# iwanders/spread_spectrum_watermarking

Measured on AMD Instinct MI355X. Metric: Mpixels/sec embed+extract (4K batch), higher is better.
Workload: dtype f64

## Files before the change

spread_spectrum_watermarking_amd/csrc/base_energy.hip:

```cpp
#include <algorithm>
#include <cmath>

#include "dct_pair_common.hpp"

namespace ssw {

namespace {

typedef _Float16 h8 __attribute__((ext_vector_type(8)));
typedef float f4 __attribute__((ext_vector_type(4)));

constexpr int BE_THREADS = 512, BE_LINES = 128;
constexpr int BE_NJ = 11;
constexpr float BE_BSCALE = 1024.0f;
constexpr unsigned BE_FRAG = 64 * 16;

struct BeClass {
    const double *x1, *x2;
    const u32x4* y16;
    const float* bmax;
    unsigned NP, Kp, pair0, pm, c1, c2, gsh, e2off, njt;
};
struct BeArgs {
    BeClass c[8];
    unsigned L, lpf, units_valid, W, chunks;
    float factor;
    float* energy;
};

__global__ __launch_bounds__(256) void base_energy_split_kernel(const double* __restrict__ y1, const double* __restrict__ y2, unsigned yrows,
                                                                unsigned NP, unsigned Kp, unsigned pair0, unsigned njt, size_t total,
                                                                _Float16* __restrict__ out, float* __restrict__ bmax) {
    const size_t idx = blockIdx.x * (size_t)blockDim.x + threadIdx.x;
    if (idx >= total) return;
    const unsigned e = (unsigned)(idx & 7u), lane = (unsigned)((idx >> 3) & 63u);
    size_t rest = idx >> 9;
    const unsigned j = (unsigned)(rest % njt);
    rest /= njt;
    const unsigned hl = (unsigned)(rest & 1u), p = (unsigned)((rest >> 1) & 1u), s = (unsigned)(rest >> 2);
    const unsigned pair = pair0 + 16u * j + (lane & 15u), k = 32u * s + 8u * (lane >> 4) + e;
    double b = 0.0;
    if (pair < NP && k < Kp) b = (p ? y2 : y1)[blk_index<double>(pair, k, yrows)];
    const float bf = (float)(b * (double)BE_BSCALE);
    const _Float16 h = (_Float16)bf;
    const float lo = bf - (float)h;
    out[idx] = hl ? (_Float16)lo : h;
    if (hl == 0 && b != 0.0) atomicMax(reinterpret_cast<unsigned*>(bmax), __float_as_uint(fabsf((float)b) * (1.0f + 0x1p-20f)));
}

__global__ __launch_bounds__(BE_THREADS) void prep16_row_energy_kernel(const BeArgs a) {
    __shared__ __attribute__((aligned(16))) u32x4 bsh[4 * BE_NJ * 64];
    __shared__ float eb[2][16 * BE_NJ];
    const unsigned tid = threadIdx.x, lane = tid & 63u, wave = tid >> 6, li = lane & 15u, lq = lane >> 4;
    const unsigned cls = blockIdx.y / a.chunks, chunk = blockIdx.y - cls * a.chunks;
    const BeClass& c = a.c[cls];
    const unsigned j0 = chunk * BE_NJ;
    if (j0 >= c.njt) return;
    const unsigned nj = c.njt - j0 < (unsigned)BE_NJ ? c.njt - j0 : (unsigned)BE_NJ;
    const unsigned m0 = blockIdx.x * BE_LINES, L = a.L;
    const unsigned z = m0 / a.lpf, unit = (m0 - z * a.lpf) / 16u + wave;
    const bool wave_valid = unit < a.units_valid && m0 + 16u * wave < L;
    const unsigned line = m0 + 16u * wave + li < L ? m0 + 16u * wave + li : L - 1u;
    const unsigned nkb = c.Kp / 8u, nsteps = (nkb + 3u) / 4u;
    for (unsigned i = tid; i < 2u * 16u * BE_NJ; i += BE_THREADS) (&eb[0][0])[i] = 0.f;

    const unsigned nq = 4u * nj * 64u;
    u32x4 breg[6];
    auto bload = [&](unsigned s) {
#pragma unroll
        for (int i = 0; i < 6; ++i) {
            const unsigned q = tid + BE_THREADS * i < nq ? tid + BE_THREADS * i : nq - 1u;
            const unsigned ph = q / (nj * 64u), rem = q - ph * (nj * 64u);
            breg[i] = c.y16[((size_t)(s * 4u + ph) * c.njt + j0) * 64u + rem];
        }
    };
    auto bstore = [&]() {
#pragma unroll
        for (int i = 0; i < 6; ++i) {
            const unsigned q = tid + BE_THREADS * i;
            if (q < nq) bsh[q] = breg[i];
        }
    };
    double2 araw[2][4];
    auto aload = [&](unsigned s) {
        const unsigned kb = 4u * s + lq;
#pragma unroll
        for (int o = 0; o < 2; ++o) {
            const double2* src = reinterpret_cast<const double2*>((o ? c.x2 : c.x1) + ((size_t)kb * L + line) * 8u);
#pragma unroll
            for (int i = 0; i < 4; ++i) araw[o][i] = kb < nkb ? src[i] : make_double2(0.0, 0.0);
        }
    };

    f4 acc[2][BE_NJ];
#pragma unroll
    for (int o = 0; o < 2; ++o)
#pragma unroll
        for (int j = 0; j < BE_NJ; ++j) acc[o][j] = (f4){0.f, 0.f, 0.f, 0.f};
    float S[2] = {0.f, 0.f};

    bload(0);
    aload(0);
    bstore();
    __syncthreads();
    for (unsigned s = 0; s < nsteps; ++s) {
        h8 xh[2], xl[2];
#pragma unroll
        for (int o = 0; o < 2; ++o)
#pragma unroll
            for (int i = 0; i < 4; ++i) {
                const float f0 = (float)araw[o][i].x, f1 = (float)araw[o][i].y;
                S[o] += fabsf(f0);
                S[o] += fabsf(f1);
                const _Float16 h0 = (_Float16)f0, h1 = (_Float16)f1;
                xh[o][2 * i] = h0; xh[o][2 * i + 1] = h1;
                xl[o][2 * i] = (_Float16)(f0 - (float)h0); xl[o][2 * i + 1] = (_Float16)(f1 - (float)h1);
            }
        if (s + 1 < nsteps) { bload(s + 1); aload(s + 1); }
        const h8* bf = reinterpret_cast<const h8*>(bsh);
#pragma unroll
        for (int j = 0; j < BE_NJ; ++j) {
            if ((unsigned)j < nj) {
#pragma unroll
            for (int o = 0; o < 2; ++o) {
                const h8 bh = bf[((2 * o) * nj + j) * 64u + lane], bl = bf[((2 * o + 1) * nj + j) * 64u + lane];
                f4 t = __builtin_amdgcn_mfma_f32_16x16x32_f16(xh[o], bl, (f4){0.f, 0.f, 0.f, 0.f}, 0, 0, 0);
                t = __builtin_amdgcn_mfma_f32_16x16x32_f16(xl[o], bh, t, 0, 0, 0);
                acc[o][j] = __builtin_amdgcn_mfma_f32_16x16x32_f16(xh[o], bh, acc[o][j], 0, 0, 0);
                acc[o][j] += t;
            }
            }
        }
        __syncthreads();
        if (s + 1 < nsteps) bstore();
        __syncthreads();
    }

#pragma unroll
    for (int o = 0; o < 2; ++o) { S[o] += __shfl_xor(S[o], 16); S[o] += __shfl_xor(S[o], 32); }
    const float k1 = 1.0f + 0x1p-20f;
    const float B = *c.bmax, n_ops = (float)(c.Kp + c.Kp / 16u + 16u);
    const float cS = (B * (3.0f * 0x1p-21f + 1.02f * n_ops * 0x1p-23f) + 0x1p-23f) * k1;
    const float cA = 1.01f * (float)c.Kp * B * 0x1p-13f * k1 + 1e-30f;
    float err[2][4];
#pragma unroll
    for (int o = 0; o < 2; ++o)
#pragma unroll
        for (int r = 0; r < 4; ++r) err[o][r] = (__shfl(S[o], (int)(4u * lq + r)) * cS + cA) * k1;
    const float fac = fabsf(a.factor) * k1;
#pragma unroll
    for (int j = 0; j < BE_NJ; ++j) {
        if ((unsigned)j >= nj) continue;
        float v1 = 0.f, v2 = 0.f;
#pragma unroll
        for (int r = 0; r < 4; ++r) {
            const float a1 = acc[0][j][r] * (1.0f / BE_BSCALE), a2 = acc[1][j][r] * (1.0f / BE_BSCALE);
            float o1, o2, e1, e2;
            if (c.pm) { o1 = fabsf(a1 + a2); o2 = fabsf(a1 - a2); e1 = e2 = err[0][r] + err[1][r]; }
            else      { o1 = fabsf(a1); o2 = fabsf(a2); e1 = err[0][r]; e2 = err[1][r]; }
            const float b1 = (o1 + e1) * k1 * fac, b2 = (o2 + e2) * k1 * fac;
            v1 += b1 * b1 * k1;
            v2 += b2 * b2 * k1;
        }
        v1 += __shfl_xor(v1, 16); v1 += __shfl_xor(v1, 32);
        v2 += __shfl_xor(v2, 16); v2 += __shfl_xor(v2, 32);
        if (wave_valid && lq == 0) {
            atomicAdd(&eb[0][16 * j + li], v1);
            atomicAdd(&eb[1][16 * j + li], v2);
        }
    }
    __syncthreads();
    if (tid < 2u * 16u * nj) {
        const unsigned o = tid / (16u * nj), pl = tid - o * (16u * nj);
        const unsigned pair = c.pair0 + 16u * j0 + pl;
        if (pair < c.NP && pair >= c.e2off * o) {
            const unsigned e = pair - (o ? c.e2off : 0u);
            const unsigned col = (o ? c.c2 : c.c1) + (e >> c.gsh) * 128u + (e & ((1u << c.gsh) - 1u));
            if (col < a.W) unsafeAtomicAdd(a.energy + (size_t)z * a.W + col, eb[o][pl]);
        }
    }
}

unsigned be_tiles(unsigned NP, unsigned pair0) { return NP > pair0 ? (NP - pair0 + 15u) / 16u : 0u; }
unsigned be_steps(unsigned Kp) { return (Kp / 8u + 3u) / 4u; }
size_t be_frag_bytes(unsigned NP, unsigned Kp, unsigned pair0) { return (size_t)be_steps(Kp) * 4u * be_tiles(NP, pair0) * BE_FRAG; }

}

size_t base_energy_split_bytes(unsigned NP, unsigned Kp, unsigned pair0) { return be_frag_bytes(NP, Kp, pair0) + 16; }

int launch_base_energy_split(hipStream_t st, const double* y1, const double* y2, unsigned yrows, unsigned NP, unsigned Kp, unsigned pair0, void* out) {
    const unsigned njt = be_tiles(NP, pair0);
    if (!y1 || !y2 || !out || njt == 0 || Kp == 0 || Kp % 8 != 0 || pair0 % 16 != 0 || yrows < NP) return SSW_ERR_BAD_ARG;
    const size_t frag = be_frag_bytes(NP, Kp, pair0), total = frag / sizeof(_Float16);
    float* bmax = reinterpret_cast<float*>(static_cast<char*>(out) + frag);
    SSW_HIP_CHECK(hipMemsetAsync(bmax, 0, 16, st));
    base_energy_split_kernel<<<(unsigned)((total + 255) / 256), 256, 0, st>>>(y1, y2, yrows, NP, Kp, pair0, njt, total, static_cast<_Float16*>(out), bmax);
    SSW_HIP_CHECK(hipGetLastError());
    return SSW_OK;
}

int launch_base_energy_bound(hipStream_t st, int n_classes, const BaseEnergyClass* cls, size_t n_frames, size_t w, size_t h, size_t lines_per_frame,
                             float factor, float* energy) {
    if (n_frames == 0 || n_classes == 0) return SSW_OK;
    const size_t lines = n_frames * lines_per_frame;
    if (n_classes < 0 || n_classes > 8 || !cls || !energy || lines_per_frame % BE_LINES != 0 || h % 16 != 0 || h > lines_per_frame ||
        lines > 0xFFFFFFFFull || w > 0xFFFFFFull || w % 128 != 0) return SSW_ERR_BAD_ARG;
    BeArgs a;
    unsigned chunks = 0;
    for (int i = 0; i < n_classes; ++i) {
        const BaseEnergyClass& s = cls[i];
        const unsigned njt = be_tiles(s.NP, s.pair0);
        if (!s.x1 || !s.x2 || !s.y16 || njt == 0 || s.Kp == 0 || s.Kp % 8 != 0 || s.pair0 % 16 != 0 || s.gsh > 16 || s.e2off > 1) return SSW_ERR_BAD_ARG;
        if ((unsigned long long)s.Kp * lines * sizeof(double) > 0xFFFFFFFFFFull) return SSW_ERR_BAD_DIMS;
        a.c[i] = BeClass{s.x1, s.x2, static_cast<const u32x4*>(s.y16),
                         reinterpret_cast<const float*>(static_cast<const char*>(s.y16) + be_frag_bytes(s.NP, s.Kp, s.pair0)),
                         s.NP, s.Kp, s.pair0, s.pm, s.c1, s.c2, s.gsh, s.e2off, njt};
        chunks = std::max(chunks, (njt + BE_NJ - 1) / BE_NJ);
    }
    a.L = (unsigned)lines; a.lpf = (unsigned)lines_per_frame; a.units_valid = (unsigned)(h / 16); a.W = (unsigned)w; a.chunks = chunks;
    a.factor = factor; a.energy = energy;
    const dim3 grid((unsigned)(lines / BE_LINES), (unsigned)n_classes * chunks);
    if (grid.y > 65535u) return SSW_ERR_BAD_DIMS;
    prep16_row_energy_kernel<<<grid, BE_THREADS, 0, st>>>(a);
    SSW_HIP_CHECK(hipGetLastError());
    return SSW_OK;
}

}
```

Baseline: 17680.

## Pipeline base-energy kernel with buffer-to-LDS DMA, double-buffered LDS and lookahead loads

Replaces the register-staged B fragment loads and LDS stores with buffer_load_lds direct-to-LDS transfers into two alternating LDS stages. X inputs are fetched via buffer loads two steps ahead, with manual waitcnt/barrier sync replacing the two __syncthreads per step. It also specializes the accumulator count by tile count (11/4/1) and software-pipelines the MFMA sequence with prefetched fragment reads. The aim is to overlap global memory latency with MFMA work and cut synchronization, at the cost of tighter 32-bit offset limits and fragile hand-written scheduling.

New measurement: 17650. No clear change (-0.1%).

```diff
diff --git a/spread_spectrum_watermarking_amd/csrc/base_energy.hip b/spread_spectrum_watermarking_amd/csrc/base_energy.hip
--- a/spread_spectrum_watermarking_amd/csrc/base_energy.hip
+++ b/spread_spectrum_watermarking_amd/csrc/base_energy.hip
@@ -1,5 +1,6 @@
 #include <algorithm>
 #include <cmath>
+#include <type_traits>
 
 #include "dct_pair_common.hpp"
 
@@ -14,12 +15,16 @@
 constexpr int BE_NJ = 11;
 constexpr float BE_BSCALE = 1024.0f;
 constexpr unsigned BE_FRAG = 64 * 16;
+constexpr int BE_AHEAD = 2;
+constexpr int BE_DMA = 6;
+constexpr unsigned BE_STAGE = 8 * BE_DMA * 64;
+constexpr unsigned BE_NONE = 0xFFFFFF00u, BE_NOFRAG = 0x80000000u;
 
 struct BeClass {
     const double *x1, *x2;
     const u32x4* y16;
     const float* bmax;
-    unsigned NP, Kp, pair0, pm, c1, c2, gsh, e2off, njt;
+    unsigned NP, Kp, pair0, pm, c1, c2, gsh, e2off, njt, ybytes;
 };
 struct BeArgs {
     BeClass c[8];
@@ -49,7 +54,9 @@
 }
 
 __global__ __launch_bounds__(BE_THREADS) void prep16_row_energy_kernel(const BeArgs a) {
-    __shared__ __attribute__((aligned(16))) u32x4 bsh[4 * BE_NJ * 64];
+#if defined(__HIP_DEVICE_COMPILE__)
+    __shared__ __attribute__((aligned(16))) u32x4 bsh0[BE_STAGE];
+    __shared__ __attribute__((aligned(16))) u32x4 bsh1[BE_STAGE];
     __shared__ float eb[2][16 * BE_NJ];
     const unsigned tid = threadIdx.x, lane = tid & 63u, wave = tid >> 6, li = lane & 15u, lq = lane >> 4;
     const unsigned cls = blockIdx.y / a.chunks, chunk = blockIdx.y - cls * a.chunks;
@@ -64,77 +71,110 @@
     const unsigned nkb = c.Kp / 8u, nsteps = (nkb + 3u) / 4u;
     for (unsigned i = tid; i < 2u * 16u * BE_NJ; i += BE_THREADS) (&eb[0][0])[i] = 0.f;
 
-    const unsigned nq = 4u * nj * 64u;
-    u32x4 breg[6];
-    auto bload = [&](unsigned s) {
-#pragma unroll
-        for (int i = 0; i < 6; ++i) {
-            const unsigned q = tid + BE_THREADS * i < nq ? tid + BE_THREADS * i : nq - 1u;
-            const unsigned ph = q / (nj * 64u), rem = q - ph * (nj * 64u);
-            breg[i] = c.y16[((size_t)(s * 4u + ph) * c.njt + j0) * 64u + rem];
-        }
-    };
-    auto bstore = [&]() {
-#pragma unroll
-        for (int i = 0; i < 6; ++i) {
-            const unsigned q = tid + BE_THREADS * i;
-            if (q < nq) bsh[q] = breg[i];
-        }
-    };
-    double2 araw[2][4];
-    auto aload = [&](unsigned s) {
+    const __amdgpu_buffer_rsrc_t yr = __builtin_amdgcn_make_buffer_rsrc((void*)c.y16, 0, c.ybytes, 0x00020000);
+    const __amdgpu_buffer_rsrc_t x1r = __builtin_amdgcn_make_buffer_rsrc((void*)c.x1, 0, nkb * L * 64u, 0x00020000);
+    const __amdgpu_buffer_rsrc_t x2r = __builtin_amdgcn_make_buffer_rsrc((void*)c.x2, 0, nkb * L * 64u, 0x00020000);
+
+    typedef __attribute__((address_space(3))) void* lds_ptr_t;
+    const unsigned wv = (unsigned)__builtin_amdgcn_readfirstlane((int)wave);
+    unsigned boff[BE_DMA];
+#pragma unroll
+    for (int i = 0; i < BE_DMA; ++i) {
+        const unsigned q = wv + 8u * i, ph = q / BE_NJ, j = q - ph * BE_NJ;
+        boff[i] = ph < 4u && j < nj ? (ph * c.njt + j0 + j) * BE_FRAG + 16u * lane : BE_NOFRAG;
+    }
+    const unsigned bstep = 4u * c.njt * BE_FRAG;
+    auto bissue = [&](unsigned s, auto stagec) {
+        u32x4* stage = decltype(stagec)::value ? bsh1 : bsh0;
+#pragma unroll
+        for (int i = 0; i < BE_DMA; ++i)
+            __builtin_amdgcn_raw_ptr_buffer_load_lds(yr, (lds_ptr_t)(&stage[(wv + 8u * i) * 64u]), 16, boff[i] + s * bstep, 0, 0, 0);
+    };
+    u32x4 araw[BE_AHEAD][2][4];
+    auto aload = [&](unsigned s, auto bufc) {
+        constexpr int ab = decltype(bufc)::value % BE_AHEAD;
         const unsigned kb = 4u * s + lq;
-#pragma unroll
-        for (int o = 0; o < 2; ++o) {
-            const double2* src = reinterpret_cast<const double2*>((o ? c.x2 : c.x1) + ((size_t)kb * L + line) * 8u);
-#pragma unroll
-            for (int i = 0; i < 4; ++i) araw[o][i] = kb < nkb ? src[i] : make_double2(0.0, 0.0);
-        }
-    };
-
-    f4 acc[2][BE_NJ];
+        const unsigned off = kb < nkb ? (kb * L + line) * 64u : BE_NONE;
+#pragma unroll
+        for (int i = 0; i < 4; ++i) {
+            araw[ab][0][i] = __builtin_amdgcn_raw_buffer_load_b128(x1r, off + 16u * i, 0, 0);
+            araw[ab][1][i] = __builtin_amdgcn_raw_buffer_load_b128(x2r, off + 16u * i, 0, 0);
+        }
+    };
+
+    auto run = [&](auto njc) {
+    constexpr int NJC = decltype(njc)::value;
+    f4 acc[2][NJC];
 #pragma unroll
     for (int o = 0; o < 2; ++o)
 #pragma unroll
-        for (int j = 0; j < BE_NJ; ++j) acc[o][j] = (f4){0.f, 0.f, 0.f, 0.f};
+        for (int j = 0; j < NJC; ++j) acc[o][j] = (f4){0.f, 0.f, 0.f, 0.f};
     float S[2] = {0.f, 0.f};
 
-    bload(0);
-    aload(0);
-    bstore();
-    __syncthreads();
-    for (unsigned s = 0; s < nsteps; ++s) {
+    using B0 = std::integral_constant<int, 0>;
+    using B1 = std::integral_constant<int, 1>;
+    auto step = [&](unsigned s, auto bufc) {
+        constexpr int buf = decltype(bufc)::value;
+        asm volatile("s_waitcnt vmcnt(%0) lgkmcnt(0)\n\ts_barrier" :: "n"(8 * (BE_AHEAD - 1)) : "memory");
+        bissue(s + 1u, std::integral_constant<int, 1 - buf>{});
+        __builtin_amdgcn_sched_barrier(0);
         h8 xh[2], xl[2];
 #pragma unroll
         for (int o = 0; o < 2; ++o)
 #pragma unroll
             for (int i = 0; i < 4; ++i) {
-                const float f0 = (float)araw[o][i].x, f1 = (float)araw[o][i].y;
+                const double2 v = __builtin_bit_cast(double2, araw[buf % BE_AHEAD][o][i]);
+                const float f0 = (float)v.x, f1 = (float)v.y;
                 S[o] += fabsf(f0);
                 S[o] += fabsf(f1);
                 const _Float16 h0 = (_Float16)f0, h1 = (_Float16)f1;
                 xh[o][2 * i] = h0; xh[o][2 * i + 1] = h1;
                 xl[o][2 * i] = (_Float16)(f0 - (float)h0); xl[o][2 * i + 1] = (_Float16)(f1 - (float)h1);
             }
-        if (s + 1 < nsteps) { bload(s + 1); aload(s + 1); }
-        const h8* bf = reinterpret_cast<const h8*>(bsh);
-#pragma unroll
-        for (int j = 0; j < BE_NJ; ++j) {
-            if ((unsigned)j < nj) {
-#pragma unroll
-            for (int o = 0; o < 2; ++o) {
-                const h8 bh = bf[((2 * o) * nj + j) * 64u + lane], bl = bf[((2 * o + 1) * nj + j) * 64u + lane];
-                f4 t = __builtin_amdgcn_mfma_f32_16x16x32_f16(xh[o], bl, (f4){0.f, 0.f, 0.f, 0.f}, 0, 0, 0);
-                t = __builtin_amdgcn_mfma_f32_16x16x32_f16(xl[o], bh, t, 0, 0, 0);
-                acc[o][j] = __builtin_amdgcn_mfma_f32_16x16x32_f16(xh[o], bh, acc[o][j], 0, 0, 0);
-                acc[o][j] += t;
-            }
-            }
-        }
-        __syncthreads();
-        if (s + 1 < nsteps) bstore();
-        __syncthreads();
-    }
+        aload(s + (unsigned)BE_AHEAD, bufc);
+        __builtin_amdgcn_sched_barrier(0);
+        const h8* bf = reinterpret_cast<const h8*>(buf ? bsh1 : bsh0) + lane;
+        constexpr int NT = 2 * NJC;
+        h8 fh[3], fl[3];
+        f4 tp = (f4){0.f, 0.f, 0.f, 0.f};
+        auto fread = [&](auto ic) {
+            constexpr int i = decltype(ic)::value, j = i / 2, o = i % 2;
+            fh[i % 3] = bf[((2 * o) * BE_NJ + j) * 64u];
+            fl[i % 3] = bf[((2 * o + 1) * BE_NJ + j) * 64u];
+        };
+        fread(std::integral_constant<int, 0>{});
+        if constexpr (NT > 1) fread(std::integral_constant<int, 1>{});
+        __builtin_amdgcn_sched_barrier(0);
+        auto term = [&](auto ic) {
+            constexpr int i = decltype(ic)::value, j = i / 2, o = i % 2;
+            if constexpr (i + 2 < NT) fread(std::integral_constant<int, i + 2>{});
+            const h8 bh = fh[i % 3], bl = fl[i % 3];
+            f4 t = __builtin_amdgcn_mfma_f32_16x16x32_f16(xh[o], bl, (f4){0.f, 0.f, 0.f, 0.f}, 0, 0, 0);
+            t = __builtin_amdgcn_mfma_f32_16x16x32_f16(xl[o], bh, t, 0, 0, 0);
+            acc[o][j] = __builtin_amdgcn_mfma_f32_16x16x32_f16(xh[o], bh, acc[o][j], 0, 0, 0);
+            if constexpr (i > 0) acc[(i - 1) % 2][(i - 1) / 2] += tp;
+            tp = t;
+            asm volatile("" : "+v"(acc[o][j]), "+v"(tp));
+            __builtin_amdgcn_sched_barrier(0);
+        };
+        auto terms = [&](auto self, auto ic) {
+            term(ic);
+            if constexpr (decltype(ic)::value + 1 < NT) self(self, std::integral_constant<int, decltype(ic)::value + 1>{});
+        };
+        terms(terms, std::integral_constant<int, 0>{});
+        acc[(NT - 1) % 2][(NT - 1) / 2] += tp;
+    };
+    aload(0u, B0{});
+    bissue(0u, B0{});
+    __builtin_amdgcn_sched_barrier(0);
+    if constexpr (BE_AHEAD == 2) aload(1u, B1{});
+    __builtin_amdgcn_sched_barrier(0);
+    for (unsigned s = 0; s + 1u < nsteps; s += 2u) {
+        step(s, B0{});
+        step(s + 1u, B1{});
+    }
+    if (nsteps & 1u) step(nsteps - 1u, B0{});
+    asm volatile("s_waitcnt vmcnt(0) lgkmcnt(0)\n\ts_barrier" ::: "memory");
 
 #pragma unroll
     for (int o = 0; o < 2; ++o) { S[o] += __shfl_xor(S[o], 16); S[o] += __shfl_xor(S[o], 32); }
@@ -149,7 +189,7 @@
         for (int r = 0; r < 4; ++r) err[o][r] = (__shfl(S[o], (int)(4u * lq + r)) * cS + cA) * k1;
     const float fac = fabsf(a.factor) * k1;
 #pragma unroll
-    for (int j = 0; j < BE_NJ; ++j) {
+    for (int j = 0; j < NJC; ++j) {
         if ((unsigned)j >= nj) continue;
         float v1 = 0.f, v2 = 0.f;
 #pragma unroll
@@ -169,6 +209,10 @@
             atomicAdd(&eb[1][16 * j + li], v2);
         }
     }
+    };
+    if (nj > 4u) run(std::integral_constant<int, BE_NJ>{});
+    else if (nj > 1u) run(std::integral_constant<int, 4>{});
+    else run(std::integral_constant<int, 1>{});
     __syncthreads();
     if (tid < 2u * 16u * nj) {
         const unsigned o = tid / (16u * nj), pl = tid - o * (16u * nj);
@@ -179,6 +223,7 @@
             if (col < a.W) unsafeAtomicAdd(a.energy + (size_t)z * a.W + col, eb[o][pl]);
         }
     }
+#endif
 }
 
 unsigned be_tiles(unsigned NP, unsigned pair0) { return NP > pair0 ? (NP - pair0 + 15u) / 16u : 0u; }
@@ -212,10 +257,11 @@
         const BaseEnergyClass& s = cls[i];
         const unsigned njt = be_tiles(s.NP, s.pair0);
         if (!s.x1 || !s.x2 || !s.y16 || njt == 0 || s.Kp == 0 || s.Kp % 8 != 0 || s.pair0 % 16 != 0 || s.gsh > 16 || s.e2off > 1) return SSW_ERR_BAD_ARG;
-        if ((unsigned long long)s.Kp * lines * sizeof(double) > 0xFFFFFFFFFFull) return SSW_ERR_BAD_DIMS;
+        const size_t frag = be_frag_bytes(s.NP, s.Kp, s.pair0);
+        if ((unsigned long long)s.Kp * lines * sizeof(double) > 0xFFFFFFFFull || frag >= BE_NOFRAG) return SSW_ERR_BAD_DIMS;
         a.c[i] = BeClass{s.x1, s.x2, static_cast<const u32x4*>(s.y16),
-                         reinterpret_cast<const float*>(static_cast<const char*>(s.y16) + be_frag_bytes(s.NP, s.Kp, s.pair0)),
-                         s.NP, s.Kp, s.pair0, s.pm, s.c1, s.c2, s.gsh, s.e2off, njt};
+                         reinterpret_cast<const float*>(static_cast<const char*>(s.y16) + frag),
+                         s.NP, s.Kp, s.pair0, s.pm, s.c1, s.c2, s.gsh, s.e2off, njt, (unsigned)frag};
         chunks = std::max(chunks, (njt + BE_NJ - 1) / BE_NJ);
     }
     a.L = (unsigned)lines; a.lpf = (unsigned)lines_per_frame; a.units_valid = (unsigned)(h / 16); a.W = (unsigned)w; a.chunks = chunks;
```
